# ginevracoal/robustBNNs

Measured on AMD Instinct MI355X. Metric: attack-samples/sec (test_pts x posterior_samples x PGD_iters), higher is better.
Workload: dtype f32 (full-width operands as three f16 pieces: 6 exact f16 MFMA product terms per fp32 product, f32 accumulate)

## Files before the change

### include/robustbnns_hip.h

```cpp
#ifndef ROBUSTBNNS_HIP_H
#define ROBUSTBNNS_HIP_H

#include <stddef.h>
#include <stdint.h>

#ifdef __cplusplus
extern "C" {
#endif

#define RBNN_ABI_VERSION 10
#define RBNN_CPAD 16

typedef enum rbnn_status {
    RBNN_OK = 0,
    RBNN_ERR_NULL = -1,
    RBNN_ERR_SHAPE = -2,
    RBNN_ERR_UNSUPPORTED = -3,
    RBNN_ERR_LAUNCH = -4,
    RBNN_ERR_ALIGN = -5
} rbnn_status;

typedef enum rbnn_activation { RBNN_ACT_RELU = 0, RBNN_ACT_LEAKY = 1, RBNN_ACT_SIGM = 2, RBNN_ACT_TANH = 3 } rbnn_activation;
typedef enum rbnn_arch { RBNN_ARCH_FC = 0, RBNN_ARCH_FC2 = 1 } rbnn_arch;

// ... 212 lines not shown
int rbnn_triple_rows(const float *src, int64_t rows, int32_t cols, int32_t ld_src, int32_t scale_exp,
                     const rbnn_dev_scale *dev_scale, void *dst, int32_t ld_dst, void *stream);

int rbnn_triple_rows_grouped(const float *src, int64_t rows, int32_t cols, int32_t ld_src, int32_t scale_exp,
                             const rbnn_dev_scale *dev_scale, void *dst, int32_t ld_dst, void *stream);

int rbnn_triple_cols(const float *W, int64_t n_mats, int32_t rows, int32_t cols, int32_t ld_src, int32_t scale_exp,
                     void *dst, int32_t ld_dst, void *stream);

int rbnn_triple_w2gen(const float *W2, int32_t n_mats, int32_t n_classes, int32_t hidden, int32_t scale_exp, void *dst,
                      void *stream);

int rbnn_fc_forward_triple(const rbnn_posterior *net, const rbnn_triple_images *tp, const rbnn_triple_workspace *tws,
                           int32_t x_exp, const rbnn_dev_scale *dev_scales, int32_t n_points, const int32_t *sample_idx,
                           int32_t n_samples, int32_t out_kind, const rbnn_workspace *ws, void *stream);

int rbnn_fc_input_grad_triple(const rbnn_posterior *net, const rbnn_triple_images *tp, const int32_t *sample_idx,
                              int32_t n_samples, int32_t n_points, int32_t chunk, const rbnn_workspace *ws,
                              const rbnn_triple_workspace *tws, int32_t *n_slabs_out, void *stream);

int rbnn_step_tail_triple(int32_t mode, const float *P, const int32_t *labels, int32_t n_samples, float inv_S, int32_t n_points,
                          int32_t n_classes, float *Psum_out, int32_t ldo, const rbnn_triple_workspace *tws, void *stream);

int rbnn_attack_step_triple(float *X, const float *X0, int32_t ldx, const float *G, int32_t n_slabs, size_t slab_stride, int32_t ldg,
                            const float *alpha, float alpha_scalar, float eps, int32_t project, int32_t n_points, int32_t in_features,
                            const rbnn_dev_scale *dev_scale, void *X_triple, int32_t ld_rows, void *stream);

typedef struct rbnn_svi_guide {
    const float *W1_loc, *W1_scale;
    const float *b1_loc, *b1_scale;
    const float *Wm_loc, *Wm_scale;
    const float *bm_loc, *bm_scale;
    const float *W2_loc, *W2_scale;
    const float *b2_loc, *b2_scale;
    int32_t hidden;
    int32_t reserved;
} rbnn_svi_guide;

#define RBNN_SVI_EPS_MAX 6.77f
int rbnn_svi_draw(const rbnn_posterior *net, const rbnn_triple_images *tp, const rbnn_svi_guide *guide, int32_t n_samples,
                  const uint64_t *sample_keys, uint64_t key, uint32_t draw_id, void *stream);
int rbnn_svi_draw_images(const rbnn_posterior *net, const rbnn_triple_images *tp, const rbnn_svi_guide *guide, int32_t n_samples,
                         const uint64_t *sample_keys, uint64_t key, uint32_t draw_id, void *stream);
int rbnn_svi_draw_supported(const rbnn_posterior *net, int32_t with_triple_images);

typedef struct rbnn_svi_flat_tensor {
// ... 116 lines not shown
```

### robustbnns_amd/_hip.py

```python
import ctypes as C
import os

import torch

_HERE = os.path.dirname(os.path.abspath(__file__))
LIB_PATH = os.path.join(_HERE, "csrc", "librbnn_hip.so")
HEADER_PATH = os.path.join(os.path.dirname(_HERE), "include", "robustbnns_hip.h")

CPAD = 16
ACTIVATIONS = {"relu": 0, "leaky": 1, "sigm": 2, "tanh": 3}
ARCHS = {"fc": 0, "fc2": 1}
OUT_PROBS, OUT_LOGITS = 0, 1
LOSS_MEAN_PROB, LOSS_PER_SAMPLE, LOSS_MEAN_LOGIT, LOSS_UPSTREAM, LOSS_UPSTREAM_LOGIT = 0, 1, 2, 3, 4

_fp = C.c_void_p


class Posterior(C.Structure):
    _fields_ = [("arch", C.c_int32), ("activation", C.c_int32), ("in_features", C.c_int32),
                ("in_stride", C.c_int32), ("hidden", C.c_int32), ("n_classes", C.c_int32),
                ("n_stored", C.c_int32), ("reserved", C.c_int32),
                ("W1", _fp), ("b1", _fp), ("Wm", _fp), ("bm", _fp), ("W2", _fp), ("b2", _fp),
                ("W1_pack4", _fp), ("Wm_pack4", _fp)]

# ... 134 lines not shown
    "rbnn_conv_forward_split": (_i32, [C.POINTER(ConvPosterior), _fp, _i32, _i32, _fp, _fp, _i32, _i32, _fp, _i32, _i32,
                                       C.POINTER(ConvWorkspace), _fp]),
    "rbnn_conv_input_grad_dense": (_i32, [C.POINTER(ConvPosterior), _fp, _i32, _f32, _fp, _i32, _i32, C.POINTER(ConvWorkspace), _fp]),
    "rbnn_conv_weight_images": (_i32, [_fp, _i32, _i32, _i32, _fp, _fp, _fp]),
    "rbnn_conv_forward_triple": (_i32, [C.POINTER(ConvPosterior), _fp, _i32, _i32, _fp, _fp, _i32, _i32, _fp, _i32, _i32,
                                        C.POINTER(ConvWorkspace), _fp]),
    "rbnn_input_scales": (_i32, [_fp, _i64, _i32, _i32, _f32, _f32, _f32, _f32, _fp, _fp]),
    "rbnn_split_rows": (_i32, [_fp, _i64, _i32, _i32, _i32, _fp, _fp, _i32, _fp]),
    "rbnn_fc_forward_split": (_i32, [_PP, C.POINTER(SplitImages), _fp, _i32, _i32, _fp, _i32, _fp, _i32, _i32, _PW, _fp]),
    "rbnn_split_cols": (_i32, [_fp, _i64, _i32, _i32, _i32, _i32, _fp, _i32, _fp]),
    "rbnn_split_w2gen": (_i32, [_fp, _i32, _i32, _i32, _i32, _fp, _fp]),
    "rbnn_split_workspace_query": (_i32, [_PP, C.POINTER(SplitImages), _i32, _i32, C.POINTER(SplitWorkspaceSizes)]),
    "rbnn_fc_input_grad_split": (_i32, [_PP, C.POINTER(SplitImages), _fp, _i32, _i32, _i32, _PW, C.POINTER(SplitWorkspace),
                                        C.POINTER(_i32), _fp]),
    "rbnn_triple_workspace_query": (_i32, [_PP, C.POINTER(TripleImages), _i32, _i32, C.POINTER(TripleWorkspaceSizes)]),
    "rbnn_triple_rows": (_i32, [_fp, _i64, _i32, _i32, _i32, _fp, _fp, _i32, _fp]),
    "rbnn_triple_rows_grouped": (_i32, [_fp, _i64, _i32, _i32, _i32, _fp, _fp, _i32, _fp]),
    "rbnn_triple_cols": (_i32, [_fp, _i64, _i32, _i32, _i32, _i32, _fp, _i32, _fp]),
    "rbnn_triple_w2gen": (_i32, [_fp, _i32, _i32, _i32, _i32, _fp, _fp]),
    "rbnn_fc_forward_triple": (_i32, [_PP, C.POINTER(TripleImages), C.POINTER(TripleWorkspace), _i32, _fp, _i32, _fp, _i32, _i32, _PW, _fp]),
    "rbnn_fc_input_grad_triple": (_i32, [_PP, C.POINTER(TripleImages), _fp, _i32, _i32, _i32, _PW, C.POINTER(TripleWorkspace),
                                         C.POINTER(_i32), _fp]),
    "rbnn_step_tail_triple": (_i32, [_i32, _fp, _fp, _i32, _f32, _i32, _i32, _fp, _i32, C.POINTER(TripleWorkspace), _fp]),
    "rbnn_attack_step_triple": (_i32, [_fp, _fp, _i32, _fp, _i32, _sz, _i32, _fp, _f32, _f32, _i32, _i32, _i32, _fp, _fp, _i32, _fp]),
    "rbnn_lowdim_supported": (_i32, [_PP]),
    "rbnn_lowdim_scratch_bytes": (_sz, [_PP, _i32, _i32]),
    "rbnn_lowdim_run": (_i32, [_PP, _i32, _i32, _i32, _fp, _fp, _i32, _i32, _fp, _i32, _fp, _f32, _f32, _f32, _fp, _f32, _i32, _i32, _i32,
                               _fp, _fp, _i32, _fp, _fp, _fp]),
    "rbnn_lowdim_fused_draw_supported": (_i32, [_PP, _i32, _i32]),
    "rbnn_lowdim_run_svi": (_i32, [_PP, C.POINTER(SviGuide), _fp, C.c_uint64, C.c_uint32, _i32, _i32, _i32, _fp, _fp, _i32, _i32, _fp, _i32, _fp, _f32,
                                   _f32, _f32, _fp, _f32, _i32, _i32, _i32, _fp, _fp, _i32, _fp, _fp, _fp]),
    "rbnn_svi_draw_flat": (_i32, [C.POINTER(SviFlatTensor), _i32, _i32, _fp, C.c_uint64, C.c_uint32, _fp]),
    "rbnn_svi_draw": (_i32, [_PP, C.POINTER(TripleImages), C.POINTER(SviGuide), _i32, _fp, C.c_uint64, C.c_uint32, _fp]),
    "rbnn_svi_draw_supported": (_i32, [_PP, _i32]),
    "rbnn_svi_draw_images": (_i32, [_PP, C.POINTER(TripleImages), C.POINTER(SviGuide), _i32, _fp, C.c_uint64, C.c_uint32, _fp]),
    "rbnn_svi_train_sizes": (_i64, [C.POINTER(SviTrainNet), C.POINTER(_i64)]),
    "rbnn_svi_train_draw": (_i32, [C.POINTER(SviTrainNet), C.c_uint64, C.c_uint32, _fp]),
    "rbnn_svi_train_forward": (_i32, [C.POINTER(SviTrainNet), _fp, _i32, _i32, _fp, C.POINTER(SviTrainWs), _fp]),
    "rbnn_svi_weight_grads": (_i32, [C.POINTER(SviTrainNet), _fp, _i32, _i32, C.POINTER(SviTrainWs), _fp]),
    "rbnn_svi_adam_step": (_i32, [C.POINTER(SviTrainNet), C.c_uint64, C.c_uint32, _i64, C.c_double, C.c_double, C.c_double, C.c_double, _fp, _fp]),
    "rbnn_svi_train_finalize": (_i32, [_fp, _i64, _fp, _i32, _fp, _i32, _fp, _i32, _fp, _fp]),
    "rbnn_nn_train_sizes": (_i64, [C.POINTER(NnTrainNet)]),
    "rbnn_nn_train_forward": (_i32, [C.POINTER(NnTrainNet), _fp, _i32, _i32, _fp, _fp, _i32, C.POINTER(NnTrainWs), _fp]),
    "rbnn_nn_weight_grads": (_i32, [C.POINTER(NnTrainNet), _fp, _i32, _i32, _fp, _i32, C.POINTER(NnTrainWs), _fp]),
    "rbnn_nn_adam_step": (_i32, [C.POINTER(NnTrainNet), _i64, C.c_double, C.c_double, C.c_double, C.c_double, _fp]),
    "rbnn_nn_train_finalize": (_i32, [C.POINTER(NnTrainNet), C.POINTER(NnTrainWs), _i32, _fp, _fp]),
    "rbnn_hmc_sizes": (_i64, [C.POINTER(SviTrainNet), C.POINTER(_i64), C.POINTER(_i64)]),
# ... 93 lines not shown
        check(self.lib.rbnn_loss_dlogits(mode, ptr(P), ptr(Psum), ldp, ptr(G_up), ptr(labels), S, inv_S, N, Cn,
                                         ptr(dZ), stream_of(P)), "rbnn_loss_dlogits")

    def fc_input_grad(self, net, sidx, S, N, chunk, ws):
        w = self._ws(ws)
        n = C.c_int32(0)
        check(self.lib.rbnn_fc_input_grad(C.byref(net.descriptor()), ptr(sidx), S, N, chunk, C.byref(w), C.byref(n),
                                          stream_of(ws["dZ"])), "rbnn_fc_input_grad")
        return n.value

    def sum_slabs(self, slabs, K, N, Dp, scale, out):
        require_gpu(slabs, "slabs")
        check(self.lib.rbnn_sum_slabs(ptr(slabs), K, N, Dp, scale, ptr(out), out.stride(0), stream_of(slabs)), "rbnn_sum_slabs")

    def sum_slabs_norms(self, slabs, K, N, Dp, D, scale, out, linf, l2):
        require_gpu(slabs, "slabs")
        check(self.lib.rbnn_sum_slabs_norms(ptr(slabs), K, N, Dp, D, scale, ptr(out), out.stride(0), ptr(linf), ptr(l2),
                                            stream_of(slabs)), "rbnn_sum_slabs_norms")

    def pgd_alpha(self, X0, D, alpha):
        require_gpu(X0, "X0")
        check(self.lib.rbnn_pgd_alpha(ptr(X0), X0.stride(0), X0.shape[0], D, ptr(alpha), stream_of(X0)), "rbnn_pgd_alpha")

    def attack_step(self, X, X0, G, K, slab_stride, ldg, alpha, alpha_scalar, eps, project, D):
        require_gpu(X, "X")
        check(self.lib.rbnn_attack_step(ptr(X), ptr(X0), X.stride(0), ptr(G), K, slab_stride, ldg, ptr(alpha),
                                        alpha_scalar, eps, int(project), X.shape[0], D, stream_of(X)), "rbnn_attack_step")

    def eval_metrics(self, A, B, labels, Cn, counts, rob):
        require_gpu(A, "outputs")
        check(self.lib.rbnn_eval_metrics(ptr(A), ptr(B), A.stride(0), ptr(labels), A.shape[0], Cn, ptr(counts), ptr(rob),
                                         stream_of(A)), "rbnn_eval_metrics")

    def pack_rows4(self, W, out):
        require_gpu(W, "W")
        cols = W.shape[-1]
        check(self.lib.rbnn_pack_rows4(ptr(W), W.numel() // cols, cols, ptr(out), stream_of(W)), "rbnn_pack_rows4")

    def input_scales(self, X, cols, floor_abs, mul, add, cap, out):
        require_gpu(X, "X")
        check(self.lib.rbnn_input_scales(ptr(X), X.shape[0], cols, X.stride(0), floor_abs, mul, add, cap, ptr(out), stream_of(X)),
              "rbnn_input_scales")
        return out

    def split_rows(self, src, cols, scale_exp, out, ld_dst, dev_scale=None):
        require_gpu(src, "src")
        ld_src = src.shape[-1]
        check(self.lib.rbnn_split_rows(ptr(src), src.numel() // ld_src, cols, ld_src, scale_exp, ptr(dev_scale), ptr(out), ld_dst,
# ... 46 lines not shown
        check(self.lib.rbnn_triple_w2gen(ptr(W2), W2.numel() // (Cn * H), Cn, H, scale_exp, ptr(out), stream_of(W2)), "rbnn_triple_w2gen")

    def triple_workspace_sizes(self, net, images, N, S):
        out = TripleWorkspaceSizes()
        check(self.lib.rbnn_triple_workspace_query(C.byref(net.descriptor(lazy_ok=True)), C.byref(images), N, S, C.byref(out)),
              "rbnn_triple_workspace_query")
        return {k: getattr(out, k) for k in TRIPLE_WS_KEYS}

    @staticmethod
    def _tws(tws):
        t = TripleWorkspace()
        for k in TRIPLE_WS_KEYS:
            setattr(t, k, ptr(tws.get(k)))
        return t

    def fc_forward_triple(self, net, images, tws, x_exp, N, sidx, S, out_kind, ws, dev_scales=None):
        w, t = self._ws(ws), self._tws(tws)
        check(self.lib.rbnn_fc_forward_triple(C.byref(net.descriptor(lazy_ok=True)), C.byref(images), C.byref(t), x_exp, ptr(dev_scales), N,
                                              ptr(sidx), S, out_kind, C.byref(w), stream_of(tws["X_triple"])), "rbnn_fc_forward_triple")

    def step_tail_triple(self, mode, P, labels, S, inv_S, N, Cn, tws, Psum=None):
        require_gpu(P, "P")
        t = self._tws(tws)
        check(self.lib.rbnn_step_tail_triple(mode, ptr(P), ptr(labels), S, inv_S, N, Cn, ptr(Psum), 0 if Psum is None else Psum.stride(0), C.byref(t),
                                             stream_of(P)), "rbnn_step_tail_triple")

    def attack_step_triple(self, X, X0, G, K, slab_stride, ldg, alpha, alpha_scalar, eps, project, D, dev_scale, X_triple, ld_rows):
        require_gpu(X, "X")
        check(self.lib.rbnn_attack_step_triple(ptr(X), ptr(X0), X.stride(0), ptr(G), K, slab_stride, ldg, ptr(alpha), alpha_scalar, eps, int(project),
                                               X.shape[0], D, ptr(dev_scale), ptr(X_triple), ld_rows, stream_of(X)), "rbnn_attack_step_triple")

    def fc_input_grad_triple(self, net, images, sidx, S, N, chunk, ws, tws, dz_ready=False):
        w, t = self._ws(ws), self._tws(tws)
        if dz_ready:
            w.dZ = None
        n = C.c_int32(0)
        check(self.lib.rbnn_fc_input_grad_triple(C.byref(net.descriptor(lazy_ok=True)), C.byref(images), ptr(sidx), S, N, chunk, C.byref(w),
                                                 C.byref(t), C.byref(n), stream_of(ws["slabs"])), "rbnn_fc_input_grad_triple")
        return n.value

    def conv_workspace_sizes(self, net, N, S):
        out = ConvWorkspaceSizes()
        check(self.lib.rbnn_conv_workspace_query(C.byref(net.descriptor()), N, S, C.byref(out)), "rbnn_conv_workspace_query")
        return {k: getattr(out, k) for k in CONV_WS_KEYS}

    @staticmethod
    def _conv_ws(ws):
        w = ConvWorkspace()
# ... 101 lines not shown
```

### robustbnns_amd/conv.py

```python
import ctypes as C
import os

import torch

from . import _hip
from .engine import AttackEngine, to_labels
from .posterior import narrow_range, scale_exp, slice_ratio, slices_in_range
from ._hip import OUT_LOGITS, OUT_PROBS

CONV_KEYS = ("model.0", "model.3", "model.7")
_U8 = {"st1", "st2"}
GEOMETRIES = {(1, 28, 28), (3, 32, 32)}


def conv_geometry(input_shape):
    p1 = (int(input_shape[1]) - 4) // 2
    return p1, p1 - 4 - 1


def range_slices(k2, k1):
    return [slice_ratio(k2, (2, 3)), slice_ratio(k2, (1, 3)), slice_ratio(k1, 2, per_sample=True)]


class ConvSviGuide:
# ... 207 lines not shown
        if self._desc is None:
            d = _hip.ConvPosterior()
            d.activation, d.hidden, d.n_classes, d.n_stored = _hip.ACTIVATIONS[self.activation], self.H, self.C, self.S
            d.in_channels, d.in_width = self.Cin, self.W
            for name, t in (("K1w", self.K1w), ("K1b", self.K1b), ("K2w", self.K2w), ("K2b", self.K2b), ("Fw", self.Fw),
                            ("Fb", self.Fb), ("K2w_ci", self.K2ci)):
                setattr(d, name, C.c_void_p(t.data_ptr()))
            self._desc = d
        return self._desc

    def state_dict(self, i):
        sd = {"model.0.weight": self.K1w[i].view(32, self.Cin, 5, 5), "model.0.bias": self.K1b[i],
              "model.3.weight": self.K2w[i].view(self.H, 32, 5, 5), "model.3.bias": self.K2b[i],
              "model.7.weight": self.Fw[i], "model.7.bias": self.Fb[i]}
        return {k: v.detach().cpu().clone() for k, v in sd.items()}


class ConvEngine(AttackEngine):

    graph_safe = False
    fused_tail = False
    pipelined_comm = False
    shared_forward = False

    def workspace(self, N, S, chunk=0, tag=0):
        key = (N, S)
        ws = self._ws_cache.get(key)
        if ws is None:
            sizes = self.k.conv_workspace_sizes(self.post, N, S)
            ws = {"n_slabs": S, "chunk": 1}
            for name in _hip.CONV_WS_KEYS:
                if name in _U8:
                    ws[name] = torch.empty(sizes[name], dtype=torch.uint8, device=self.device)
                else:
                    ws[name] = torch.empty(sizes[name] // 4, dtype=torch.float32, device=self.device)
            ws["slabs"] = ws["G"]
            ws["Psum"] = torch.zeros(N, _hip.CPAD, dtype=torch.float32, device=self.device)
            ws["Gsum"] = torch.empty(N, self.post.D, dtype=torch.float32, device=self.device)
            while len(self._ws_cache) >= 2:
                self._ws_cache.pop(next(iter(self._ws_cache)))
            self._ws_cache[key] = ws
        return ws

    def point_block(self, S):
        p = self.post
        p1 = 32 * p.P1W * p.P1W
# ... 78 lines not shown
```

### robustbnns_amd/csrc/rbnn_kernels.hip

```cpp
#include "rbnn_common.hpp"
#include <stdlib.h>

namespace {

struct FwdArgs {
    const float* X;   long long x_sample_stride;  int ldx;  int N;
    const float* W;   long long w_sample_stride;  int ldw;  int KT;
    const float* b;
    const float* W2;  const float* b2;            int C;    int H;
    const int* sidx;  int S;   int NT;
    float* P;  uint32_t* mask;  float* dact;  float* hid;  int out_kind;
};

template <int ACT, int WH, int HTW, int WN, int NTW, bool LAYER2>
__global__ void __launch_bounds__(64 * WH * WN, (HTW * NTW > 16 ? 2 : (WH * WN) / 2)) fc_forward_kernel(const FwdArgs a) {
    constexpr int BH = WH * HTW * 16, BN = WN * NTW * 16;
    constexpr int TILE = (BH + BN) * 16;
    constexpr bool BITMASK = (ACT == RBNN_ACT_RELU || ACT == RBNN_ACT_LEAKY);
    constexpr int NW = WH * WN;
    static_assert(NW == 4 || NW == 8, "4 or 8 waves per block");
    static_assert(HTW % 2 == 0 && HTW <= 8, "a wave's h range is whole 32-bit mask words, at most 4");
    static_assert(WH * BN * 16 <= 2 * TILE, "the Z^T reduction scratch aliases the tile buffers");
    __shared__ __attribute__((aligned(16))) float lds[2 * TILE];
    float* const zred = lds;
// ... 468 lines not shown

__global__ void attack_step4_kernel(float* __restrict__ X, const float* __restrict__ X0, int ldx,
                                    const float* __restrict__ G, int K, long long slab_stride, int ldg,
                                    const float* __restrict__ alpha, float alpha_scalar, float eps, int project,
                                    int N, int D4) {
    const long long i = (long long)blockIdx.x * blockDim.x + threadIdx.x;
    if (i >= (long long)N * D4) return;
    const long long n = i / D4;
    const int d = 4 * (int)(i % D4);
    f32x4 g = *(const f32x4*)(G + n * ldg + d);
    for (int k = 1; k < K; ++k) g += *(const f32x4*)(G + k * slab_stride + n * ldg + d);
    const float step = alpha ? alpha[n] : alpha_scalar;
    const f32x4 x = *(const f32x4*)(X + n * ldx + d);
    f32x4 x0 = x, out;
    if (project) x0 = *(const f32x4*)(X0 + n * ldx + d);
#pragma unroll
    for (int r = 0; r < 4; ++r) {
        const float sgn = (g[r] > 0.f) ? 1.f : ((g[r] < 0.f) ? -1.f : 0.f);
        float pert = x[r] + step * sgn;
        if (project) pert = x0[r] + fminf(fmaxf(pert - x0[r], -eps), eps);
        out[r] = fminf(fmaxf(pert, 0.f), 1.f);
    }
    *(f32x4*)(X + n * ldx + d) = out;
}

__global__ void eval_metrics_kernel(const float* __restrict__ A, const float* __restrict__ B, int ldp,
                                    const int* __restrict__ labels, int N, int C, int* __restrict__ counts,
                                    float* __restrict__ rob) {
    const int n = blockIdx.x * blockDim.x + threadIdx.x;
    int ok_a = 0, ok_b = 0;
    if (n < N) {
        float ma = -INFINITY, mb = -INFINITY;
        int ia = 0, ib = 0;
        for (int c = 0; c < C; ++c) {
            const float a = A[(long long)n * ldp + c], b = B[(long long)n * ldp + c];
            if (a > ma) { ma = a; ia = c; }
            if (b > mb) { mb = b; ib = c; }
        }
        float da = 0.f, db = 0.f;
        for (int c = 0; c < C; ++c) { da += expf(A[(long long)n * ldp + c] - ma); db += expf(B[(long long)n * ldp + c] - mb); }
        float diff = 0.f;
        for (int c = 0; c < C; ++c)
            diff = fmaxf(diff, fabsf(expf(A[(long long)n * ldp + c] - ma) / da - expf(B[(long long)n * ldp + c] - mb) / db));
        rob[n] = 1.f - diff;
        ok_a = (ia == labels[n]);
        ok_b = (ib == labels[n]);
// ... 297 lines not shown
int rbnn_pgd_alpha(const float* X0, int32_t ldx, int32_t N, int32_t D, float* alpha, void* stream) {
    if (!X0 || !alpha) return RBNN_ERR_NULL;
    if (N < 1 || D < 1 || ldx < D) return RBNN_ERR_SHAPE;
    hipLaunchKernelGGL(pgd_alpha_kernel, dim3((N + 3) / 4), dim3(256), 0, (hipStream_t)stream, X0, ldx, N, D, alpha);
    return launch_status();
}

int rbnn_attack_step(float* X, const float* X0, int32_t ldx, const float* G, int32_t K, size_t slab_stride, int32_t ldg,
                     const float* alpha, float alpha_scalar, float eps, int32_t project, int32_t N, int32_t D, void* stream) {
    if (!X || !G || (project && !X0)) return RBNN_ERR_NULL;
    if (N < 1 || D < 1 || ldx < D || ldg < D || K < 1) return RBNN_ERR_SHAPE;
    if (!(D & 3) && !(ldx & 3) && !(ldg & 3) && !(slab_stride & 3) && aligned16(X) && aligned16(G) && (!project || aligned16(X0))) {
        const long long total4 = (long long)N * (D / 4);
        hipLaunchKernelGGL(attack_step4_kernel, dim3((unsigned)((total4 + 255) / 256)), dim3(256), 0, (hipStream_t)stream,
                           X, X0, ldx, G, K, (long long)slab_stride, ldg, alpha, alpha_scalar, eps, project, N, D / 4);
        return launch_status();
    }
    const long long total = (long long)N * D;
    hipLaunchKernelGGL(attack_step_kernel, dim3((unsigned)((total + 255) / 256)), dim3(256), 0, (hipStream_t)stream,
                       X, X0, ldx, G, K, (long long)slab_stride, ldg, alpha, alpha_scalar, eps, project, N, D);
    return launch_status();
}

int rbnn_eval_metrics(const float* out_orig, const float* out_adv, int32_t ldp, const int32_t* labels, int32_t N, int32_t C,
                      int32_t* counts, float* rob, void* stream) {
    if (!out_orig || !out_adv || !labels || !counts || !rob) return RBNN_ERR_NULL;
    if (N < 1 || C < 1 || ldp < C) return RBNN_ERR_SHAPE;
    if (hipMemsetAsync(counts, 0, 2 * sizeof(int32_t), (hipStream_t)stream) != hipSuccess) return RBNN_ERR_LAUNCH;
    hipLaunchKernelGGL(eval_metrics_kernel, dim3((N + 255) / 256), dim3(256), 0, (hipStream_t)stream,
                       out_orig, out_adv, ldp, labels, N, C, counts, rob);
    return launch_status();
}

int rbnn_pack_rows4(const float* W, int64_t rows, int32_t cols, float* out, void* stream) {
    if (!W || !out) return RBNN_ERR_NULL;
    if (rows < 4 || (rows & 3) || cols < 1) return RBNN_ERR_SHAPE;
    if (!aligned16(out)) return RBNN_ERR_ALIGN;
    const long long total = (rows / 4) * (long long)cols;
    hipLaunchKernelGGL(pack_rows4_kernel, dim3((unsigned)((total + 255) / 256)), dim3(256), 0, (hipStream_t)stream, W, (long long)(rows / 4), cols, out);
    return launch_status();
}

int rbnn_svi_materialize(const float* loc, const float* scale_raw, const float* eps, int64_t n_elem, int32_t S, float* out, void* stream) {
    if (!loc || !scale_raw || !eps || !out) return RBNN_ERR_NULL;
    if (n_elem < 1 || S < 1) return RBNN_ERR_SHAPE;
    const long long total = (long long)n_elem * S;
// ... 7 lines not shown
```

### robustbnns_amd/csrc/rbnn_triple.hip

```cpp
#include "rbnn_common.hpp"
#include <algorithm>
#include <cstdlib>

namespace {

__device__ __forceinline__ void split3(float v, _Float16& p0, _Float16& p1, _Float16& p2) {
    p0 = (_Float16)v;
    float r = v - (float)p0;
    p1 = (_Float16)r;
    r -= (float)p1;
    p2 = (_Float16)r;
}

#ifndef RBNN_X3_PAIR_NOP
#define RBNN_X3_PAIR_NOP 0
#endif
#if RBNN_X3_PAIR_NOP
#define RBNN_X3_PAIR_PAD "\n\ts_nop 1"
#else
#define RBNN_X3_PAIR_PAD ""
#endif
#define RBNN_X3_PAIR_BODY \
    "v_bfe_i32 %[me], %[mw], %[b0], 1\n\t" \
    "v_bfe_i32 %[mo], %[mw], %[b1], 1\n\t" \
// ... 560 lines not shown
    for (int s = q; s < S; s += 16) {
        _Float16 d[3][10];
        float dz[16];
#pragma unroll
        for (int c = 0; c < 16; ++c) dz[c] = 0.f;
        if (n < N) tail_dz<MODE>(P + ((long long)s * N + n) * RBNN_CPAD, gmean, y, C, inv_S, dz);
#pragma unroll
        for (int c = 0; c < 10; ++c) {
            const float x = (n < N && c < C) ? ldexpf(dz[c], e) : 0.f;
            split3(x, d[0][c], d[1][c], d[2][c]);
        }
        uint4* const o = dst + ((long long)s * N_pad + n) * 4;
#pragma unroll
        for (int ch = 0; ch < 3; ++ch) {
            union { f16x8 v; uint4 u; } w;
#pragma unroll
            for (int j = 0; j < 8; ++j) w.v[j] = d[ch][j];
            o[ch ^ sw] = w.u;
        }
        union { f16x8 v; uint4 u; } t;
        t.v[0] = d[0][8]; t.v[1] = d[0][9]; t.v[2] = d[1][8]; t.v[3] = d[1][9];
        t.v[4] = d[2][8]; t.v[5] = d[2][9]; t.v[6] = d[0][8]; t.v[7] = d[0][9];
        o[3 ^ sw] = t.u;
    }
}

__global__ void __launch_bounds__(256) attack_step_x3_kernel(float* __restrict__ X, const float* __restrict__ X0, int ldx, const float* __restrict__ G,
                                                             int K, long long slab_stride, int ldg, const float* __restrict__ alpha, float alpha_scalar,
                                                             float eps, int project, long long N, int D, const rbnn_dev_scale* __restrict__ ds,
                                                             uint4* __restrict__ dst, int groups) {
    const long long i = (long long)blockIdx.x * blockDim.x + threadIdx.x;
    if (i >= N * groups) return;
    const long long n = i / groups;
    const int gq = (int)(i % groups), d0 = 8 * gq;
    const float scale = ds->scale;
    float xn[8];
#pragma unroll
    for (int j = 0; j < 8; ++j) xn[j] = 0.f;
    if (d0 < D) {
        const float step = alpha ? alpha[n] : alpha_scalar;
#pragma unroll
        for (int h = 0; h < 2; ++h) {
            const int d = d0 + 4 * h;
            if (d < D) {
                f32x4 g = *(const f32x4*)(G + n * ldg + d);
                for (int k = 1; k < K; ++k) g += *(const f32x4*)(G + k * slab_stride + n * ldg + d);
// ... 428 lines not shown
    b.x_ds = dev_scales ? dev_scales + 1 : nullptr; b.hid_ds = nullptr;
    b.mask = ws->mask2; b.dact = ws->dact2; b.hid = nullptr;
    return launch_forward_x3<true, true>(net->activation, b, st);
}

int rbnn_step_tail_triple(int32_t mode, const float* P, const int32_t* labels, int32_t S, float inv_S, int32_t N, int32_t C, float* Psum_out,
                          int32_t ldo, const rbnn_triple_workspace* tws, void* stream) {
    if (!P || !labels || !tws || !tws->dZ_gen || !tws->g_scale) return RBNN_ERR_NULL;
    if (mode != RBNN_LOSS_MEAN_PROB && mode != RBNN_LOSS_PER_SAMPLE && mode != RBNN_LOSS_MEAN_LOGIT) return RBNN_ERR_UNSUPPORTED;
    if (S < 1 || N < 1 || C < 1 || C > 10 || (Psum_out && ldo < C)) return RBNN_ERR_SHAPE;
    if (!aligned16(P) || !aligned16(tws->dZ_gen)) return RBNN_ERR_ALIGN;
    const long long n_pad = mask_ld(N);
    const dim3 grid((unsigned)(n_pad / 16)), block(256);
    hipStream_t st = (hipStream_t)stream;
    if (mode == RBNN_LOSS_MEAN_PROB)
        hipLaunchKernelGGL(step_tail_x3_kernel<RBNN_LOSS_MEAN_PROB>, grid, block, 0, st, P, labels, S, inv_S, N, n_pad, C, Psum_out, ldo, (uint4*)tws->dZ_gen, tws->g_scale);
    else if (mode == RBNN_LOSS_PER_SAMPLE)
        hipLaunchKernelGGL(step_tail_x3_kernel<RBNN_LOSS_PER_SAMPLE>, grid, block, 0, st, P, labels, S, inv_S, N, n_pad, C, Psum_out, ldo, (uint4*)tws->dZ_gen, tws->g_scale);
    else
        hipLaunchKernelGGL(step_tail_x3_kernel<RBNN_LOSS_MEAN_LOGIT>, grid, block, 0, st, P, labels, S, inv_S, N, n_pad, C, Psum_out, ldo, (uint4*)tws->dZ_gen, tws->g_scale);
    return launch_status();
}

int rbnn_attack_step_triple(float* X, const float* X0, int32_t ldx, const float* G, int32_t K, size_t slab_stride, int32_t ldg, const float* alpha,
                            float alpha_scalar, float eps, int32_t project, int32_t N, int32_t D, const rbnn_dev_scale* dev_scale, void* X_triple,
                            int32_t ld_rows, void* stream) {
    if (!X || !G || (project && !X0) || !dev_scale || !X_triple) return RBNN_ERR_NULL;
    if (N < 1 || D < 1 || ldx < D || ldg < D || K < 1 || ld_rows < D || (ld_rows & 31)) return RBNN_ERR_SHAPE;
    if ((D & 3) || (ldx & 3) || (ldg & 3) || (slab_stride & 3)) return RBNN_ERR_SHAPE;
    if (!aligned16(X) || !aligned16(G) || (project && !aligned16(X0)) || !aligned16(X_triple)) return RBNN_ERR_ALIGN;
    const int groups = ld_rows / 8;
    const long long total = (long long)N * groups;
    hipLaunchKernelGGL(attack_step_x3_kernel, dim3((unsigned)((total + 255) / 256)), dim3(256), 0, (hipStream_t)stream,
                       X, X0, ldx, G, K, (long long)slab_stride, ldg, alpha, alpha_scalar, eps, project, (long long)N, D, dev_scale, (uint4*)X_triple, groups);
    return launch_status();
}

int rbnn_fc_input_grad_triple(const rbnn_posterior* net, const rbnn_triple_images* tp, const int32_t* sidx, int32_t S,
                              int32_t N, int32_t chunk, const rbnn_workspace* ws, const rbnn_triple_workspace* tws,
                              int32_t* n_slabs_out, void* stream) {
    if (!net || !tp || !ws || !tws || !ws->slabs) return RBNN_ERR_NULL;
    if (!tp->W1_cols || !tp->W2_gen || !tws->dZ_gen || !tws->g_scale) return RBNN_ERR_NULL;
    if (net->arch != RBNN_ARCH_FC && net->arch != RBNN_ARCH_FC2) return RBNN_ERR_UNSUPPORTED;
    if (net->activation < RBNN_ACT_RELU || net->activation > RBNN_ACT_TANH) return RBNN_ERR_UNSUPPORTED;
    const bool fc2 = net->arch == RBNN_ARCH_FC2, bm = net->activation == RBNN_ACT_RELU || net->activation == RBNN_ACT_LEAKY;
    if (bm ? !ws->mask1 : !ws->dact1) return RBNN_ERR_NULL;
// ... 49 lines not shown
```

### robustbnns_amd/engine.py

```python
import os

import torch

from . import _hip
from ._hip import (LOSS_MEAN_LOGIT, LOSS_MEAN_PROB, LOSS_PER_SAMPLE, LOSS_UPSTREAM, LOSS_UPSTREAM_LOGIT, OUT_LOGITS, OUT_PROBS)

_WS_DTYPE = {"mask1": torch.int32, "mask2": torch.int32}


def to_labels(y, device):
    y = torch.as_tensor(y)
    if y.dim() >= 2:
        y = y.argmax(-1)
    return y.to(device=device, dtype=torch.int32).contiguous()


class _DifferentiableForward(torch.autograd.Function):

    @staticmethod
    def forward(ctx, x, engine, sidx, S, logits):
        ctx.engine, ctx.sidx, ctx.S, ctx.logits = engine, sidx, S, logits
        ctx.save_for_backward(x.detach())
        out = engine.forward_padded(engine.pad_inputs(x), sidx, S, OUT_LOGITS if logits else OUT_PROBS)
        return out[:, :engine.post.C].clone()
# ... 354 lines not shown
        N, p = Xp.shape[0], self.post
        G = ws["Gsum"] if "Gsum" in ws else ws["G"]
        if norms is not None and self.world == 1:
            self.k.sum_slabs_norms(ws["slabs"], n_slabs, N, p.Dp, p.D, scale, G, norms[0], norms[1])
            return G
        self.k.sum_slabs(ws["slabs"], n_slabs, N, p.Dp, scale, G)
        self._allreduce(G)
        if norms is not None:
            out = torch.empty_like(G)
            self.k.sum_slabs_norms(G, 1, N, p.Dp, p.D, 1.0, out, norms[0], norms[1])
            return out
        return G

    def loss_gradients(self, x, y, n_samples, seeds=None, norms=False):
        sidx, S = self.sample_index(n_samples, seeds)
        nb = None
        if norms:
            nb = (torch.empty(x.shape[0], dtype=torch.float32, device=self.device),
                  torch.empty(x.shape[0], dtype=torch.float32, device=self.device))
        xin = self._flat(x) if self.precision == "lowdim" else self.pad_inputs(x)
        G = self.gradient(xin, to_labels(y, self.device), sidx, S, LOSS_PER_SAMPLE, norms=nb)
        return (self.unpad(G, x), nb[0], nb[1]) if norms else self.unpad(G, x)

    def _step(self, X, X0, labels, sidx, S, mode, alpha, alpha_scalar, eps, project):
        p = self.post
        if self.world > 1 and self.pipelined_comm:
            return self._step_sharded(X, X0, labels, sidx, S, mode, alpha, alpha_scalar, eps, project)
        ws, n_slabs, _ = self.gradient_slabs(X, labels, sidx, S, mode)
        if (self.world == 1 and self._carry_image and self._fused_tail(mode, None) and self._scales is not None and "triple" in ws
                and p.D % 4 == 0):
            self.k.attack_step_triple(X, X0, ws["slabs"], n_slabs, X.shape[0] * p.Dp, p.Dp, alpha, alpha_scalar, eps, project, p.D,
                                      self._scales, ws["triple"]["X_triple"], self.post.triple_images().ld_rows)
            ws["x_image_ready"] = X.data_ptr()
        elif self.world == 1:
            self.k.attack_step(X, X0, ws["slabs"], n_slabs, X.shape[0] * p.Dp, p.Dp, alpha, alpha_scalar, eps, project, p.D)
        else:
            G = ws["Gsum"] if "Gsum" in ws else ws["G"]
            self.k.sum_slabs(ws["slabs"], n_slabs, X.shape[0], p.Dp, 1.0, G)
            self._allreduce(G)
            self.k.attack_step(X, X0, G, 1, 0, p.Dp, alpha, alpha_scalar, eps, project, p.D)

    pipelined_comm = True

    def _comm_blocks(self, N, S=None):
        env = os.environ.get("RBNN_COMM_BLOCKS")
        if env is not None:
            want = int(env)
        else:
            want = 2 if (S is not None and S * getattr(self.post, "Hp", 1 << 30) < 16384) else 1
        return max(1, min(want, N // max(1, int(os.environ.get("RBNN_COMM_MIN_POINTS", "512")))))

    def _step_sharded(self, X, X0, labels, sidx, S, mode, alpha, alpha_scalar, eps, project):
        p, N, C = self.post, X.shape[0], self.post.C
        nb = self._comm_blocks(N, S)
        bounds = [0] + [min(N, (N * i // nb + 255) // 256 * 256) for i in range(1, nb)] + [N]
        bounds = sorted(set(bounds))
# ... 9 lines not shown
            h = None
            if need_psum:
                self.k.reduce_samples(ws["P"], S, hi - lo, C, 1.0, ws["Psum"])
                h = self._allreduce_async(ws["Psum"])
            blocks.append((lo, hi, ws, h))
        pending = []
        for lo, hi, ws, h in blocks:
            if h is not None:
                self._wait(h)
            self.k.loss_dlogits(mode, ws["P"], ws["Psum"] if need_psum else None, None, labels[lo:hi], S, inv_S, hi - lo, C, ws["dZ"])
            n_slabs = self._grad_kernels(sidx, S, hi - lo, ws)
            self.k.sum_slabs(ws["slabs"], n_slabs, hi - lo, p.Dp, 1.0, ws["G"])
            pending.append(self._allreduce_async(ws["G"]))
        for (lo, hi, ws, _), h in zip(blocks, pending):
            self._wait(h)
            self.k.attack_step(X[lo:hi], None if X0 is None else X0[lo:hi], ws["G"], 1, 0, p.Dp,
                               None if alpha is None else alpha[lo:hi], alpha_scalar, eps, project, p.D)

    def fgsm(self, x, y, n_samples, epsilon=0.3, seeds=None, mode=LOSS_MEAN_PROB):
        sidx, S = self.sample_index(n_samples, seeds)
        if self.precision == "lowdim":
            out = self._lowdim_attack(self._flat(x), None, to_labels(y, self.device), sidx, S, mode, None, 0.0, False, float(epsilon), False, 1)
            return out.reshape(x.shape)
        X = self.pad_inputs(x, clone=True)
        self._scales = self._input_scales(X, iterates=False)
        try:
            self._step(X, None, to_labels(y, self.device), sidx, S, mode, None, float(epsilon), 0.0, False)
        finally:
            self._scales = None
        return self.unpad(X, x)

    def attack_gradient(self, x, y, n_samples, seeds=None, mode=LOSS_MEAN_PROB):
        sidx, S = self.sample_index(n_samples, seeds)
        xin = self._flat(x) if self.precision == "lowdim" else self.pad_inputs(x)
        return self.gradient(xin, to_labels(y, self.device), sidx, S, mode).clone()

    def fgsm_from_gradient(self, x, G, epsilon):
        p = self.post
        X = self.pad_inputs(x, clone=True)
        self.k.attack_step(X, None, G, 1, 0, p.Dp, None, float(epsilon), 0.0, False, p.D)
        return self.unpad(X, x)

    shared_forward = True

    def loss_gradients_and_fgsm(self, x, y, n_samples, epsilon=0.3, seeds=None, mode=LOSS_MEAN_PROB):
        if not self.shared_forward or self.precision == "lowdim" or mode != LOSS_MEAN_PROB:
            return self.loss_gradients(x, y, n_samples, seeds), self.fgsm(x, y, n_samples, epsilon, seeds, mode)
        sidx, S = self.sample_index(n_samples, seeds)
        labels = to_labels(y, self.device)
        p = self.post
        X = self.pad_inputs(x, clone=True)
        N = X.shape[0]
        self._scales = self._input_scales(X, iterates=False)
# ... 154 lines not shown
```

Baseline: 134.7 million.

## Add streamed step-tail kernel and out-of-place FGSM step avoiding input clone

Adds a new streamed step-tail kernel for the triple-precision path. It computes the per-point probability sum, the dz max-scale and the split f16 dz image in one launch, and it becomes the default through an env switch. Separately, FGSM on contiguous unpadded inputs now skips the padded clone and writes the perturbed result to a fresh output buffer through a new out-of-place step kernel. The cost is that the tail kernel reads P several times and recomputes the softmax gradient in two passes, which may not beat the old multi-kernel tail.

Result: no change. 135.4 million (median of 6 runs) (+0.5%).

```diff
diff --git a/include/robustbnns_hip.h b/include/robustbnns_hip.h
--- a/include/robustbnns_hip.h
+++ b/include/robustbnns_hip.h
@@ -258,6 +258,12 @@
 int rbnn_step_tail_triple(int32_t mode, const float *P, const int32_t *labels, int32_t n_samples, float inv_S, int32_t n_points,
                           int32_t n_classes, float *Psum_out, int32_t ldo, const rbnn_triple_workspace *tws, void *stream);
 
+int rbnn_step_tail_triple_stream(int32_t mode, const float *P, const int32_t *labels, int32_t n_samples, float inv_S, int32_t n_points,
+                                 int32_t n_classes, float *Psum_out, int32_t ldo, const rbnn_triple_workspace *tws, void *stream);
+
+int rbnn_fgsm_step_out(const float *X, float *X_out, int32_t ldx, const float *G, int32_t n_slabs, size_t slab_stride, int32_t ldg,
+                       float eps, int32_t n_points, int32_t in_features, void *stream);
+
 int rbnn_attack_step_triple(float *X, const float *X0, int32_t ldx, const float *G, int32_t n_slabs, size_t slab_stride, int32_t ldg,
                             const float *alpha, float alpha_scalar, float eps, int32_t project, int32_t n_points, int32_t in_features,
                             const rbnn_dev_scale *dev_scale, void *X_triple, int32_t ld_rows, void *stream);
diff --git a/robustbnns_amd/_hip.py b/robustbnns_amd/_hip.py
--- a/robustbnns_amd/_hip.py
+++ b/robustbnns_amd/_hip.py
@@ -180,7 +180,9 @@
     "rbnn_fc_input_grad_triple": (_i32, [_PP, C.POINTER(TripleImages), _fp, _i32, _i32, _i32, _PW, C.POINTER(TripleWorkspace),
                                          C.POINTER(_i32), _fp]),
     "rbnn_step_tail_triple": (_i32, [_i32, _fp, _fp, _i32, _f32, _i32, _i32, _fp, _i32, C.POINTER(TripleWorkspace), _fp]),
+    "rbnn_step_tail_triple_stream": (_i32, [_i32, _fp, _fp, _i32, _f32, _i32, _i32, _fp, _i32, C.POINTER(TripleWorkspace), _fp]),
     "rbnn_attack_step_triple": (_i32, [_fp, _fp, _i32, _fp, _i32, _sz, _i32, _fp, _f32, _f32, _i32, _i32, _i32, _fp, _fp, _i32, _fp]),
+    "rbnn_fgsm_step_out": (_i32, [_fp, _fp, _i32, _fp, _i32, _sz, _i32, _f32, _i32, _i32, _fp]),
     "rbnn_lowdim_supported": (_i32, [_PP]),
     "rbnn_lowdim_scratch_bytes": (_sz, [_PP, _i32, _i32]),
     "rbnn_lowdim_run": (_i32, [_PP, _i32, _i32, _i32, _fp, _fp, _i32, _i32, _fp, _i32, _fp, _f32, _f32, _f32, _fp, _f32, _i32, _i32, _i32,
@@ -320,8 +322,15 @@
         require_gpu(X0, "X0")
         check(self.lib.rbnn_pgd_alpha(ptr(X0), X0.stride(0), X0.shape[0], D, ptr(alpha), stream_of(X0)), "rbnn_pgd_alpha")
 
-    def attack_step(self, X, X0, G, K, slab_stride, ldg, alpha, alpha_scalar, eps, project, D):
-        require_gpu(X, "X")
+    def attack_step(self, X, X0, G, K, slab_stride, ldg, alpha, alpha_scalar, eps, project, D, out=None):
+        require_gpu(X, "X")
+        if out is not None:
+            if project or alpha is not None or X0 is not None or out.stride(0) != X.stride(0):
+                raise HipError("attack_step(out=...) is the plain FGSM step: no projection, a scalar step, X and out of one row stride")
+            require_gpu(out, "out")
+            check(self.lib.rbnn_fgsm_step_out(ptr(X), ptr(out), X.stride(0), ptr(G), K, slab_stride, ldg, alpha_scalar, X.shape[0], D, stream_of(X)),
+                  "rbnn_fgsm_step_out")
+            return
         check(self.lib.rbnn_attack_step(ptr(X), ptr(X0), X.stride(0), ptr(G), K, slab_stride, ldg, ptr(alpha),
                                         alpha_scalar, eps, int(project), X.shape[0], D, stream_of(X)), "rbnn_attack_step")
 
@@ -414,8 +423,9 @@
     def step_tail_triple(self, mode, P, labels, S, inv_S, N, Cn, tws, Psum=None):
         require_gpu(P, "P")
         t = self._tws(tws)
-        check(self.lib.rbnn_step_tail_triple(mode, ptr(P), ptr(labels), S, inv_S, N, Cn, ptr(Psum), 0 if Psum is None else Psum.stride(0), C.byref(t),
-                                             stream_of(P)), "rbnn_step_tail_triple")
+        name = "rbnn_step_tail_triple" if os.environ.get("RBNN_TAIL_STREAM", "1") == "0" else "rbnn_step_tail_triple_stream"
+        check(getattr(self.lib, name)(mode, ptr(P), ptr(labels), S, inv_S, N, Cn, ptr(Psum), 0 if Psum is None else Psum.stride(0), C.byref(t),
+                                      stream_of(P)), name)
 
     def attack_step_triple(self, X, X0, G, K, slab_stride, ldg, alpha, alpha_scalar, eps, project, D, dev_scale, X_triple, ld_rows):
         require_gpu(X, "X")
diff --git a/robustbnns_amd/conv.py b/robustbnns_amd/conv.py
--- a/robustbnns_amd/conv.py
+++ b/robustbnns_amd/conv.py
@@ -253,6 +253,7 @@
     fused_tail = False
     pipelined_comm = False
     shared_forward = False
+    out_of_place_fgsm = False
 
     def workspace(self, N, S, chunk=0, tag=0):
         key = (N, S)
diff --git a/robustbnns_amd/csrc/rbnn_kernels.hip b/robustbnns_amd/csrc/rbnn_kernels.hip
--- a/robustbnns_amd/csrc/rbnn_kernels.hip
+++ b/robustbnns_amd/csrc/rbnn_kernels.hip
@@ -514,6 +514,25 @@
         out[r] = fminf(fmaxf(pert, 0.f), 1.f);
     }
     *(f32x4*)(X + n * ldx + d) = out;
+}
+
+__global__ void fgsm_step4_out_kernel(const float* __restrict__ X, float* __restrict__ Xout, int ldx,
+                                      const float* __restrict__ G, int K, long long slab_stride, int ldg, float step, int N, int D4) {
+    const long long i = (long long)blockIdx.x * blockDim.x + threadIdx.x;
+    if (i >= (long long)N * D4) return;
+    const long long n = i / D4;
+    const int d = 4 * (int)(i % D4);
+    f32x4 g = *(const f32x4*)(G + n * ldg + d);
+    for (int k = 1; k < K; ++k) g += *(const f32x4*)(G + k * slab_stride + n * ldg + d);
+    const f32x4 x = *(const f32x4*)(X + n * ldx + d);
+    f32x4 out;
+#pragma unroll
+    for (int r = 0; r < 4; ++r) {
+        const float sgn = (g[r] > 0.f) ? 1.f : ((g[r] < 0.f) ? -1.f : 0.f);
+        const float pert = x[r] + step * sgn;
+        out[r] = fminf(fmaxf(pert, 0.f), 1.f);
+    }
+    *(f32x4*)(Xout + n * ldx + d) = out;
 }
 
 __global__ void eval_metrics_kernel(const float* __restrict__ A, const float* __restrict__ B, int ldp,
@@ -857,6 +876,18 @@
     return launch_status();
 }
 
+int rbnn_fgsm_step_out(const float* X, float* X_out, int32_t ldx, const float* G, int32_t K, size_t slab_stride, int32_t ldg, float eps,
+                       int32_t N, int32_t D, void* stream) {
+    if (!X || !X_out || !G) return RBNN_ERR_NULL;
+    if (N < 1 || D < 1 || ldx < D || ldg < D || K < 1 || X == X_out) return RBNN_ERR_SHAPE;
+    if ((D & 3) || (ldx & 3) || (ldg & 3) || (slab_stride & 3)) return RBNN_ERR_SHAPE;
+    if (!aligned16(X) || !aligned16(X_out) || !aligned16(G)) return RBNN_ERR_ALIGN;
+    const long long total4 = (long long)N * (D / 4);
+    hipLaunchKernelGGL(fgsm_step4_out_kernel, dim3((unsigned)((total4 + 255) / 256)), dim3(256), 0, (hipStream_t)stream,
+                       X, X_out, ldx, G, K, (long long)slab_stride, ldg, eps, N, D / 4);
+    return launch_status();
+}
+
 int rbnn_eval_metrics(const float* out_orig, const float* out_adv, int32_t ldp, const int32_t* labels, int32_t N, int32_t C,
                       int32_t* counts, float* rob, void* stream) {
     if (!out_orig || !out_adv || !labels || !counts || !rob) return RBNN_ERR_NULL;
diff --git a/robustbnns_amd/csrc/rbnn_triple.hip b/robustbnns_amd/csrc/rbnn_triple.hip
--- a/robustbnns_amd/csrc/rbnn_triple.hip
+++ b/robustbnns_amd/csrc/rbnn_triple.hip
@@ -606,6 +606,149 @@
         t.v[0] = d[0][8]; t.v[1] = d[0][9]; t.v[2] = d[1][8]; t.v[3] = d[1][9];
         t.v[4] = d[2][8]; t.v[5] = d[2][9]; t.v[6] = d[0][8]; t.v[7] = d[0][9];
         o[3 ^ sw] = t.u;
+    }
+}
+
+constexpr int TAIL_UA = 16, TAIL_UC = 4;
+
+template <int MODE>
+__device__ __forceinline__ void tail_dz_rows(const f32x4 (&v)[4], const float (&gmean)[16], int y, int C, float inv_S, float (&out)[16]) {
+    float p[16], g[16];
+#pragma unroll
+    for (int q = 0; q < 4; ++q)
+#pragma unroll
+        for (int r = 0; r < 4; ++r) p[4 * q + r] = v[q][r];
+    if (MODE == RBNN_LOSS_PER_SAMPLE) {
+        ce_softmax_grad<16>(p, C, y, inv_S, g);
+    } else {
+#pragma unroll
+        for (int c = 0; c < 16; ++c) g[c] = gmean[c];
+    }
+    if (MODE == RBNN_LOSS_MEAN_LOGIT) {
+#pragma unroll
+        for (int c = 0; c < 16; ++c) out[c] = g[c];
+    } else {
+        softmax_backward<16>(g, p, C, out);
+    }
+}
+
+template <int MODE>
+__global__ void __launch_bounds__(256) streamed_step_tail_x3_kernel(const float* __restrict__ P, const int* __restrict__ labels, int S, float inv_S, int N,
+                                                                  long long N_pad, int C, float* __restrict__ Psum_out, int ldo,
+                                                                  uint4* __restrict__ dst, float* __restrict__ gscale) {
+    __shared__ float red[16][17];
+    __shared__ float psum[16][16];
+    const int p = threadIdx.x & 15, q = threadIdx.x >> 4;
+    const long long n = (long long)blockIdx.x * 16 + p;
+    const long long row = (long long)N * RBNN_CPAD;
+    if (MODE != RBNN_LOSS_PER_SAMPLE) {
+        if (q < 4) {
+            f32x4 sum = (f32x4){0.f, 0.f, 0.f, 0.f};
+            if (n < N) {
+                const float* src = P + n * RBNN_CPAD + 4 * q;
+                int s = 0;
+                for (; s + TAIL_UA <= S; s += TAIL_UA, src += TAIL_UA * row) {
+                    f32x4 v[TAIL_UA];
+#pragma unroll
+                    for (int j = 0; j < TAIL_UA; ++j) v[j] = *(const f32x4*)(src + j * row);
+#pragma unroll
+                    for (int j = 0; j < TAIL_UA; ++j) sum += v[j];
+                }
+                if (s < S) {
+                    f32x4 v[TAIL_UA];
+#pragma unroll
+                    for (int j = 0; j < TAIL_UA; ++j) if (s + j < S) v[j] = *(const f32x4*)(src + j * row);
+#pragma unroll
+                    for (int j = 0; j < TAIL_UA; ++j) if (s + j < S) sum += v[j];
+                }
+            }
+#pragma unroll
+            for (int r = 0; r < 4; ++r) {
+                psum[p][4 * q + r] = sum[r];
+                if (Psum_out && n < N && 4 * q + r < C) Psum_out[n * ldo + 4 * q + r] = sum[r];
+            }
+        }
+        __syncthreads();
+    }
+    const int y = (n < N) ? labels[n] : 0;
+    float gmean[16];
+    if (MODE != RBNN_LOSS_PER_SAMPLE) {
+        float t[16];
+#pragma unroll
+        for (int c = 0; c < 16; ++c) t[c] = (c < C) ? psum[p][c] * inv_S : 0.f;
+        ce_softmax_grad<16>(t, C, y, inv_S, gmean);
+    } else {
+#pragma unroll
+        for (int c = 0; c < 16; ++c) gmean[c] = 0.f;
+    }
+    float m = 0.f;
+    if (n < N)
+        for (int s0 = q; s0 < S; s0 += 16 * TAIL_UC) {
+            f32x4 v[TAIL_UC][4];
+#pragma unroll
+            for (int j = 0; j < TAIL_UC; ++j)
+                if (s0 + 16 * j < S) {
+                    const float* const src = P + (s0 + 16 * j) * row + n * RBNN_CPAD;
+#pragma unroll
+                    for (int k = 0; k < 4; ++k) v[j][k] = *(const f32x4*)(src + 4 * k);
+                }
+#pragma unroll
+            for (int j = 0; j < TAIL_UC; ++j)
+                if (s0 + 16 * j < S) {
+                    float dz[16];
+                    tail_dz_rows<MODE>(v[j], gmean, y, C, inv_S, dz);
+#pragma unroll
+                    for (int c = 0; c < 12; ++c) if (c < C) m = fmaxf(m, fabsf(dz[c]));
+                }
+        }
+    red[q][p] = m;
+    __syncthreads();
+    m = 0.f;
+#pragma unroll
+    for (int i = 0; i < 16; ++i) m = fmaxf(m, red[i][p]);
+    int e = 0;
+    if (m > 0.f && m < INFINITY) e = min(13 - ilogbf(m), 120);
+    if (q == 0) gscale[n] = ldexpf(1.f, -e);
+    const int sw = dz_swz3(n);
+    for (int s0 = q; s0 < S; s0 += 16 * TAIL_UC) {
+        f32x4 v[TAIL_UC][4];
+        if (n < N) {
+#pragma unroll
+            for (int j = 0; j < TAIL_UC; ++j)
+                if (s0 + 16 * j < S) {
+                    const float* const src = P + (s0 + 16 * j) * row + n * RBNN_CPAD;
+#pragma unroll
+                    for (int k = 0; k < 4; ++k) v[j][k] = *(const f32x4*)(src + 4 * k);
+                }
+        }
+#pragma unroll
+        for (int j = 0; j < TAIL_UC; ++j) {
+            const int s = s0 + 16 * j;
+            if (s < S) {
+                _Float16 d[3][10];
+                float dz[16];
+#pragma unroll
+                for (int c = 0; c < 16; ++c) dz[c] = 0.f;
+                if (n < N) tail_dz_rows<MODE>(v[j], gmean, y, C, inv_S, dz);
+#pragma unroll
+                for (int c = 0; c < 10; ++c) {
+                    const float x = (n < N && c < C) ? ldexpf(dz[c], e) : 0.f;
+                    split3(x, d[0][c], d[1][c], d[2][c]);
+                }
+                uint4* const o = dst + ((long long)s * N_pad + n) * 4;
+#pragma unroll
+                for (int ch = 0; ch < 3; ++ch) {
+                    union { f16x8 v; uint4 u; } w;
+#pragma unroll
+                    for (int jj = 0; jj < 8; ++jj) w.v[jj] = d[ch][jj];
+                    o[ch ^ sw] = w.u;
+                }
+                union { f16x8 v; uint4 u; } t;
+                t.v[0] = d[0][8]; t.v[1] = d[0][9]; t.v[2] = d[1][8]; t.v[3] = d[1][9];
+                t.v[4] = d[2][8]; t.v[5] = d[2][9]; t.v[6] = d[0][8]; t.v[7] = d[0][9];
+                o[3 ^ sw] = t.u;
+            }
+        }
     }
 }
 
@@ -1080,6 +1223,24 @@
     return launch_status();
 }
 
+int rbnn_step_tail_triple_stream(int32_t mode, const float* P, const int32_t* labels, int32_t S, float inv_S, int32_t N, int32_t C, float* Psum_out,
+                                 int32_t ldo, const rbnn_triple_workspace* tws, void* stream) {
+    if (!P || !labels || !tws || !tws->dZ_gen || !tws->g_scale) return RBNN_ERR_NULL;
+    if (mode != RBNN_LOSS_MEAN_PROB && mode != RBNN_LOSS_PER_SAMPLE && mode != RBNN_LOSS_MEAN_LOGIT) return RBNN_ERR_UNSUPPORTED;
+    if (S < 1 || N < 1 || C < 1 || C > 10 || (Psum_out && ldo < C)) return RBNN_ERR_SHAPE;
+    if (!aligned16(P) || !aligned16(tws->dZ_gen)) return RBNN_ERR_ALIGN;
+    const long long n_pad = mask_ld(N);
+    const dim3 grid((unsigned)(n_pad / 16)), block(256);
+    hipStream_t st = (hipStream_t)stream;
+    if (mode == RBNN_LOSS_MEAN_PROB)
+        hipLaunchKernelGGL(streamed_step_tail_x3_kernel<RBNN_LOSS_MEAN_PROB>, grid, block, 0, st, P, labels, S, inv_S, N, n_pad, C, Psum_out, ldo, (uint4*)tws->dZ_gen, tws->g_scale);
+    else if (mode == RBNN_LOSS_PER_SAMPLE)
+        hipLaunchKernelGGL(streamed_step_tail_x3_kernel<RBNN_LOSS_PER_SAMPLE>, grid, block, 0, st, P, labels, S, inv_S, N, n_pad, C, Psum_out, ldo, (uint4*)tws->dZ_gen, tws->g_scale);
+    else
+        hipLaunchKernelGGL(streamed_step_tail_x3_kernel<RBNN_LOSS_MEAN_LOGIT>, grid, block, 0, st, P, labels, S, inv_S, N, n_pad, C, Psum_out, ldo, (uint4*)tws->dZ_gen, tws->g_scale);
+    return launch_status();
+}
+
 int rbnn_attack_step_triple(float* X, const float* X0, int32_t ldx, const float* G, int32_t K, size_t slab_stride, int32_t ldg, const float* alpha,
                             float alpha_scalar, float eps, int32_t project, int32_t N, int32_t D, const rbnn_dev_scale* dev_scale, void* X_triple,
                             int32_t ld_rows, void* stream) {
diff --git a/robustbnns_amd/engine.py b/robustbnns_amd/engine.py
--- a/robustbnns_amd/engine.py
+++ b/robustbnns_amd/engine.py
@@ -400,7 +400,7 @@
         G = self.gradient(xin, to_labels(y, self.device), sidx, S, LOSS_PER_SAMPLE, norms=nb)
         return (self.unpad(G, x), nb[0], nb[1]) if norms else self.unpad(G, x)
 
-    def _step(self, X, X0, labels, sidx, S, mode, alpha, alpha_scalar, eps, project):
+    def _step(self, X, X0, labels, sidx, S, mode, alpha, alpha_scalar, eps, project, out=None):
         p = self.post
         if self.world > 1 and self.pipelined_comm:
             return self._step_sharded(X, X0, labels, sidx, S, mode, alpha, alpha_scalar, eps, project)
@@ -410,6 +410,8 @@
             self.k.attack_step_triple(X, X0, ws["slabs"], n_slabs, X.shape[0] * p.Dp, p.Dp, alpha, alpha_scalar, eps, project, p.D,
                                       self._scales, ws["triple"]["X_triple"], self.post.triple_images().ld_rows)
             ws["x_image_ready"] = X.data_ptr()
+        elif self.world == 1 and out is not None:
+            self.k.attack_step(X, X0, ws["slabs"], n_slabs, X.shape[0] * p.Dp, p.Dp, alpha, alpha_scalar, eps, project, p.D, out=out)
         elif self.world == 1:
             self.k.attack_step(X, X0, ws["slabs"], n_slabs, X.shape[0] * p.Dp, p.Dp, alpha, alpha_scalar, eps, project, p.D)
         else:
@@ -465,6 +467,15 @@
         if self.precision == "lowdim":
             out = self._lowdim_attack(self._flat(x), None, to_labels(y, self.device), sidx, S, mode, None, 0.0, False, float(epsilon), False, 1)
             return out.reshape(x.shape)
+        X = self._fgsm_source(x)
+        if X is not None:
+            out = torch.empty_like(X)
+            self._scales = self._input_scales(X, iterates=False)
+            try:
+                self._step(X, None, to_labels(y, self.device), sidx, S, mode, None, float(epsilon), 0.0, False, out=out)
+            finally:
+                self._scales = None
+            return out.reshape(x.shape)
         X = self.pad_inputs(x, clone=True)
         self._scales = self._input_scales(X, iterates=False)
         try:
@@ -472,6 +483,18 @@
         finally:
             self._scales = None
         return self.unpad(X, x)
+
+    out_of_place_fgsm = True
+
+    def _fgsm_source(self, x):
+        p = self.post
+        if not (self.out_of_place_fgsm and self.precision == "triple" and self.world == 1 and isinstance(self.k, _hip.HipKernels)
+                and p.Dp == p.D and p.D % 4 == 0 and os.environ.get("RBNN_FGSM_OUT", "1") != "0"):
+            return None
+        if not torch.is_tensor(x) or not x.is_contiguous() or x.dim() < 2 or x.shape[0] < 1 or x.numel() != x.shape[0] * p.D:
+            return None
+        xf = x.detach().reshape(x.shape[0], -1).to(self.device, torch.float32)
+        return xf if xf.is_contiguous() and xf.data_ptr() % 16 == 0 else None
 
     def attack_gradient(self, x, y, n_samples, seeds=None, mode=LOSS_MEAN_PROB):
         sidx, S = self.sample_index(n_samples, seeds)
```
